# LiMeng95/MultiPoseNet.pytorch

Measured on AMD Instinct MI355X. Metric: images/sec (train fwd+bwd) ResNet101 480x480 bs=32/GPU, higher is better.
Workload: dtype bf16; 1 GPU; R101 full posenet (keypoint+detection) train step: fwd + MSE/focal losses + bwd + Adam, 480x480, 32 images/GPU, bf16 MFMA / fp32 accumulate / fp32 master weights; global_batch=32, parallelism=dp1, loss_log=asynchronous (set_lazy_log), launch=recorded launch list re-issued per step (replay.py), 87 replays, optimizer_update=Adam in one launch after backward

## Files before the change

### include/mpn.h

```cpp
#ifndef MPN_H_
#define MPN_H_
#include <stdint.h>

#ifdef __cplusplus
extern "C" {
#endif

#define MPN_F32 0
#define MPN_BF16 1
#define MPN_F16 2

#define MPN_E_BADARG (-2)
#define MPN_E_UNSUPPORTED (-3)

typedef struct MpnConvParams {
    const void* x;
    const void* w;
    void* y;
    const float* bias;
    const float* scale;
    const void* res;
    const uint8_t* res_mask;
    float* stats;
    int64_t x_sB, x_sH, x_sW;
// ... 51 lines not shown
    const void* dy;
    float* dw;
    float* ws;
    int64_t x_sB, x_sH, x_sW;
    int64_t dy_sP;
    int32_t B, H, W, Cin;
    int32_t Ho, Wo, Cout;
    int32_t R, S, stride, pad;
    int32_t dtype;
    int32_t chunks;
    float* db;
    float* db_ws;
    int32_t nseg;
    int32_t seg_H[5], seg_W[5];
    int32_t seg_chunk0[6];
    int32_t seg_chunk_pixels;
    const void* seg_x[5];
    const void* seg_dy[5];
    int32_t kseg_n, kseg_c;
    int32_t kseg_shift[4];
    const void* kseg_x[4];
} MpnWgradParams;
int mpn_debug_wgrad_prof(void* buf);
int mpn_debug_igemm_prof(void* buf);

int mpn_conv_wgrad_chunks(const MpnWgradParams* p);
int mpn_conv_wgrad_seg_plan(MpnWgradParams* p);
int mpn_conv_wgrad(const MpnWgradParams* p, void* stream);
int mpn_conv_wgrad_partials(const MpnWgradParams* p, void* stream);
int mpn_conv_wgrad_reduce(const MpnWgradParams* p, void* stream);
int mpn_conv_wgrad_kernel_id(const MpnWgradParams* p);
int mpn_conv_wgrad_kernel_name(const MpnWgradParams* p, char* buf, int cap);

int mpn_reduce_partials(const float* ws, int chunks, int64_t n, float* dst, int accumulate, void* stream);

int mpn_cast_f32_to_bf16(const float* src, void* dst, int64_t n, void* stream);
int mpn_cast_f32(const float* src, void* dst, int64_t n, int dtype, void* stream);
int mpn_weight_transpose(const float* w, void* wt, int Cout, int RS, int Cin, int Cout_pad,
                         int dtype, void* stream);
int mpn_weight_transpose_batched(const float* arena, void* dst, const int64_t* table, int nlayers, int64_t nblocks,
                                 int dtype, void* stream);
int mpn_weight_pad_k(const float* w, void* dst, int Cout, int K, int Kpad, int dtype, void* stream);
int mpn_stem_pack_weight(const float* w, void* packed, int Cout, int dtype, void* stream);
int mpn_stem_unpack_wgrad(const float* dpacked, float* dw, int Cout, void* stream);
int mpn_stem_pack_image(const float* img, int64_t sB, int64_t sC, int64_t sH, int64_t sW, void* dst,
                        int B, int H, int W, int dtype, void* stream);

int mpn_bn_finalize_train(const float* stats, int tiles, int C, int64_t count, const float* gamma,
                          const float* beta, float* running_mean, float* running_var, float momentum,
                          float eps, float* mean, float* invstd, float* scale, float* shift, void* stream);
int mpn_bn_finalize_eval(int C, const float* gamma, const float* beta, const float* running_mean,
                         const float* running_var, float eps, float* mean, float* invstd,
                         float* scale, float* shift, void* stream);
int mpn_bn_act_forward(const void* y, const void* res, void* z, const float* scale, const float* shift,
                       int64_t P, int C, int Cs, int relu, int dtype, uint8_t* mask, void* stream);
int mpn_bn_bwd_reduce(const void* dz, const void* z, const void* y, const float* mean, const float* invstd,
                      const float* mask_scale, const float* mask_shift, float* partial, int chunks, int64_t P, int C, int Cs, int relu, int dtype, void* stream);
int mpn_bn_bwd_finalize(const float* partial, int chunks, int C, int64_t count, const float* gamma, const float* mean,
                        const float* invstd, int train, float* dgamma, float* dbeta, float* coef, void* stream);
int mpn_bn_bwd_apply(const void* dz, const void* z, const void* y, const float* k1, const float* k2, const float* k3,
                     const float* mask_scale, const float* mask_shift, void* dy, void* dres, int dres_accumulate, int64_t P, int C, int Cs, int relu, int dtype,
                     const uint8_t* mask, void* stream);
int mpn_bn_bwd_chunks(int64_t P, int Cs, int dtype);

int mpn_maxpool3x3s2_forward(const void* x, void* y, uint8_t* idx, int B, int H, int W, int Cs,
                             int Ho, int Wo, int dtype, void* stream);
// ... 162 lines not shown
```

### multiposenet/pytorch_amd/_lib.py

```python
import ctypes
import os
import subprocess

import torch

_HERE = os.path.dirname(os.path.abspath(__file__))
LIB_PATH = os.path.join(_HERE, "libmpn_hip.so")
CSRC = os.path.join(_HERE, "csrc")

F32, BF16, F16 = 0, 1, 2


class MpnError(RuntimeError):
    pass


class ConvParams(ctypes.Structure):
    _fields_ = [
        ("x", ctypes.c_void_p), ("w", ctypes.c_void_p), ("y", ctypes.c_void_p),
        ("bias", ctypes.c_void_p), ("scale", ctypes.c_void_p), ("res", ctypes.c_void_p), ("res_mask", ctypes.c_void_p),
        ("stats", ctypes.c_void_p),
        ("x_sB", ctypes.c_int64), ("x_sH", ctypes.c_int64), ("x_sW", ctypes.c_int64),
        ("y_sB", ctypes.c_int64), ("y_sP", ctypes.c_int64),
        ("res_sB", ctypes.c_int64), ("res_sP", ctypes.c_int64),
# ... 29 lines not shown
        ("seg_chunk_pixels", ctypes.c_int32), ("seg_x", ctypes.c_void_p * 5), ("seg_dy", ctypes.c_void_p * 5),
        ("kseg_n", ctypes.c_int32), ("kseg_c", ctypes.c_int32), ("kseg_shift", ctypes.c_int32 * 4), ("kseg_x", ctypes.c_void_p * 4),
    ]


_vp, _i, _i64, _f = ctypes.c_void_p, ctypes.c_int, ctypes.c_int64, ctypes.c_float
_PC = ctypes.POINTER(ConvParams)
_PW = ctypes.POINTER(WgradParams)

SIGNATURES = {
    "mpn_gt_heatmaps": (_i, [_vp, _vp, _i, _i, _vp, _i, _i, ctypes.c_double, ctypes.c_double, _vp]),
    "mpn_augment_image": (_i, [_vp, _i64, _vp, _i, _vp, _i, _i, ctypes.POINTER(ctypes.c_float), _vp]),
    "mpn_augment_mask": (_i, [_vp, _i64, _vp, _i, _vp, _i, _i, _i, _i, _vp]),
    "mpn_prn_train_maps": (_i, [_vp, _vp, _vp, _vp, _i, _i, _i, ctypes.c_double, _vp, _vp, _vp, _vp, _vp, _vp]),
    "mpn_heatmap_peaks_workspace_bytes": (_i64, [_i, _i, _i, _i, _i]),
    "mpn_heatmap_peaks": (_i, [_vp, _i64, _i64, _i64, _i64, _i, _i, _i, _i, _f, ctypes.c_double, _i, _vp, _vp, _i, _vp, _vp]),
    "mpn_resize": (_i, [_vp, _i64, _i64, _i64, _i, _i, _i, _vp, _i, _i, _i, ctypes.c_double, ctypes.c_double, _vp]),
    "mpn_prn_build_maps": (_i, [_vp, _vp, _vp, _vp, _i, _i, _i, ctypes.c_double, _vp, _vp, _vp, _vp, _vp]),
    "mpn_prn_scores": (_i, [_vp, _vp, _i, _i, _i, _i, _vp, _vp, _vp]),
    "mpn_prn_scores_compact": (_i, [_vp, _vp, _i, _i, _i, _i, _i, _vp, _vp, _vp, _vp, _vp, _vp]),
    "mpn_prn_match_host": (_i, [_i, _vp, _vp, _vp, _vp, _vp, _vp, _vp, _i, _vp, _i, _i, _vp, _vp]),
    "mpn_conv_stats_tiles": (_i, [_PC]),
    "mpn_conv_kernel_name": (_i, [_PC, ctypes.c_char_p, _i]),
    "mpn_conv_forward": (_i, [_PC, _vp]),
    "mpn_debug_wgrad_prof": (_i, [_vp]),
    "mpn_debug_igemm_prof": (_i, [_vp]),
    "mpn_conv_wgrad_chunks": (_i, [_PW]),
    "mpn_conv_wgrad_seg_plan": (_i, [_PW]),
    "mpn_conv_wgrad": (_i, [_PW, _vp]),
    "mpn_conv_wgrad_partials": (_i, [_PW, _vp]),
    "mpn_conv_wgrad_reduce": (_i, [_PW, _vp]),
    "mpn_conv_wgrad_kernel_id": (_i, [_PW]),
    "mpn_conv_wgrad_kernel_name": (_i, [_PW, ctypes.c_char_p, _i]),
    "mpn_reduce_partials": (_i, [_vp, _i, _i64, _vp, _i, _vp]),
    "mpn_cast_f32_to_bf16": (_i, [_vp, _vp, _i64, _vp]),
    "mpn_cast_f32": (_i, [_vp, _vp, _i64, _i, _vp]),
    "mpn_weight_transpose": (_i, [_vp, _vp, _i, _i, _i, _i, _i, _vp]),
    "mpn_weight_transpose_batched": (_i, [_vp, _vp, _vp, _i, _i64, _i, _vp]),
    "mpn_weight_pad_k": (_i, [_vp, _vp, _i, _i, _i, _i, _vp]),
    "mpn_stem_pack_weight": (_i, [_vp, _vp, _i, _i, _vp]),
    "mpn_stem_unpack_wgrad": (_i, [_vp, _vp, _i, _vp]),
    "mpn_stem_pack_image": (_i, [_vp, _i64, _i64, _i64, _i64, _vp, _i, _i, _i, _i, _vp]),
    "mpn_bn_finalize_train": (_i, [_vp, _i, _i, _i64, _vp, _vp, _vp, _vp, _f, _f, _vp, _vp, _vp, _vp, _vp]),
    "mpn_bn_finalize_eval": (_i, [_i, _vp, _vp, _vp, _vp, _f, _vp, _vp, _vp, _vp, _vp]),
    "mpn_bn_act_forward": (_i, [_vp, _vp, _vp, _vp, _vp, _i64, _i, _i, _i, _i, _vp, _vp]),
    "mpn_bn_bwd_reduce": (_i, [_vp, _vp, _vp, _vp, _vp, _vp, _vp, _vp, _i, _i64, _i, _i, _i, _i, _vp]),
    "mpn_bn_bwd_finalize": (_i, [_vp, _i, _i, _i64, _vp, _vp, _vp, _i, _vp, _vp, _vp, _vp]),
    "mpn_bn_bwd_apply": (_i, [_vp, _vp, _vp, _vp, _vp, _vp, _vp, _vp, _vp, _vp, _i, _i64, _i, _i, _i, _i, _vp, _vp]),
    "mpn_bn_bwd_chunks": (_i, [_i64, _i, _i]),
    "mpn_maxpool3x3s2_forward": (_i, [_vp, _vp, _vp, _i, _i, _i, _i, _i, _i, _i, _vp]),
    "mpn_maxpool3x3s2_backward": (_i, [_vp, _vp, _vp, _i, _i, _i, _i, _i, _i, _i, _vp]),
    "mpn_upsample_nearest_backward": (_i, [_vp, _vp, _i, _i, _i, _i, _i, _i, _i, _i, _vp]),
    "mpn_upsample_nearest_slice": (_i, [_vp, _vp, _i, _i, _i, _i, _i, _i, _i, _i, _i, _vp]),
    "mpn_upsample_nearest_slice_backward": (_i, [_vp, _vp, _i, _i, _i, _i, _i, _i, _i, _i, _i, _vp]),
    "mpn_export_f32": (_i, [_vp, _i, _vp, _i, _i, _i, _i, _i, _i, _i, _i64, _i64, _vp]),
    "mpn_import_grad": (_i, [_vp, _i64, _i64, _vp, _i, _i, _i, _i, _i, _i, _i, _i, _vp]),
    "mpn_nchw_to_nhwc_f32": (_i, [_vp, _i64, _i64, _i64, _i64, _vp, _i, _i, _i, _i, _vp]),
    "mpn_det_pack": (_i, [_vp, _i, _vp, _i, _i64, _i, _i, _i64, _vp]),
    "mpn_det_unpack": (_i, [_vp, _vp, _i, _i, _i64, _i, _i, _i64, _vp]),
    "mpn_relu_forward": (_i, [_vp, _vp, _i64, _i, _vp]),
    "mpn_relu_backward": (_i, [_vp, _vp, _vp, _i64, _i, _i, _vp]),
    "mpn_add_inplace": (_i, [_vp, _vp, _i64, _i, _vp]),
    "mpn_channel_sum": (_i, [_vp, _i, _i64, _i, _i, _vp, _i, _vp]),
    "mpn_colsum_rows": (_i, [_vp, _i, _i64, _i, _i, _vp, _vp]),
    "mpn_channel_sum_chunks": (_i, [_i64, _i, _i]),
    "mpn_mse_chunks": (_i, [_i64]),
# ... 20 lines not shown
    "mpn_box_decode_clip": (_i, [_vp, _vp, _vp, _i, _i, _f, _f, _vp]),
    "mpn_box_decode_clip_ms": (_i, [_vp, _vp, _vp, _i, _i, _f, _f, ctypes.POINTER(ctypes.c_float), _vp]),
    "mpn_clip_boxes": (_i, [_vp, _i64, _f, _f, _vp]),
    "mpn_score_filter": (_i, [_vp, _vp, _i, _f, _vp, _vp, _vp, _vp]),
    "mpn_score_filter_batched": (_i, [_vp, _vp, _i, _i, _f, _vp, _vp, _vp, _vp]),
    "mpn_gather_dets_batched": (_i, [_vp, _i64, _vp, _i64, _vp, _i, _i, _vp, _vp, _i64, _vp]),
    "mpn_gather_class": (_i, [_vp, _vp, _i, _vp, _i64, _vp, _i, _i, _vp, _i64, _vp]),
    "mpn_nms_batched_workspace_bytes": (_i64, [_i, _i64]),
    "mpn_nms_batched": (_i, [_vp, _i64, _vp, _i, _i64, _f, _i, _vp, _i64, _vp, _vp, _vp]),
    "mpn_nms_batched_topk": (_i, [_vp, _i64, _vp, _i, _i64, _i64, _f, _i, _vp, _i64, _vp, _vp, _vp]),
    "mpn_nms_workspace_bytes": (_i64, [_i64]),
    "mpn_nms": (_i, [_vp, _i64, _f, _i, _vp, _vp, _vp, _vp]),
    "mpn_adam_step": (_i, [_vp, _vp, _vp, _vp, _i64, _f, _f, _f, _f, _f, _f, _f, _f, _vp]),
    "mpn_adam_advance": (_i, [_vp, _vp]),
    "mpn_adam_step_dev": (_i, [_vp, _vp, _vp, _vp, _i64, _vp, _vp]),
    "mpn_grad_absmax_workspace_bytes": (_i64, [_i64]),
    "mpn_grad_absmax_partial": (_i, [_vp, _i64, _vp, _vp]),
    "mpn_grad_clip_finalize": (_i, [_vp, _i64, _vp, _vp, _vp, _vp]),
    "mpn_adam_step_clip_dev": (_i, [_vp, _vp, _vp, _vp, _i64, _vp, _vp, _vp]),
    "mpn_scale_by_dev": (_i, [_vp, _i64, _vp, _vp]),
    "mpn_fill_f32": (_i, [_vp, _f, _i64, _vp]),
    "mpn_copy_bytes": (_i, [_vp, _vp, _i64, _vp]),
    "mpn_step_log": (_i, [_vp, _vp, _vp, _vp]),
    "mpn_conv2cls_comb_elems": (_i64, [_i, _i]),
    "mpn_conv2cls_combine": (_i, [_vp, _vp, _i, _i, _vp]),
    "mpn_conv2cls_expand": (_i, [_vp, _vp, _vp, _i, _i, _i, _i, _i, _vp]),
    "mpn_conv2cls_classsum": (_i, [_vp, _vp, _i, _i, _i, _i, _vp]),
    "mpn_conv2cls_pool": (_i, [_vp, _vp, _vp, _i, _i, _i, _i, _i, _vp]),
    "mpn_conv2cls_tapsum": (_i, [_vp, _vp, _i, _i, _i, _i, _i, _vp]),
    "mpn_conv2cls_fold": (_i, [_vp, _vp, _i, _i, _vp]),
    "mpn_version": (ctypes.c_char_p, []),
}

_COUNT_FUNCS = {"mpn_conv_stats_tiles", "mpn_conv_kernel_name", "mpn_conv_wgrad_chunks", "mpn_conv_wgrad_seg_plan", "mpn_conv_wgrad_kernel_id", "mpn_conv_wgrad_kernel_name", "mpn_bn_bwd_chunks", "mpn_channel_sum_chunks",
                "mpn_mse_chunks", "mpn_mse_train_blocks", "mpn_focal_blocks", "mpn_focal_mc_blocks", "mpn_bce_chunks", "mpn_nms_workspace_bytes", "mpn_nms_batched_workspace_bytes", "mpn_heatmap_peaks_workspace_bytes", "mpn_conv2cls_comb_elems", "mpn_grad_absmax_workspace_bytes", "mpn_version"}

_lib = None


def build(force=False):
    if force and os.path.exists(LIB_PATH):
        os.remove(LIB_PATH)
    subprocess.check_call(["make", "-s", "-j8", "-C", CSRC])
    if not os.path.exists(LIB_PATH):
        raise MpnError("build did not produce %s" % LIB_PATH)
    return LIB_PATH


def use_experiments_build():
    global LIB_PATH
    assert _lib is None, "call use_experiments_build() before anything loads the library"
    subprocess.check_call(["make", "-s", "-j8", "-C", CSRC, "experiments"])
    LIB_PATH = os.path.join(_HERE, "libmpn_hip_experiments.so")
    return LIB_PATH


def lib():
    global _lib
    if _lib is None:
        if not os.path.exists(LIB_PATH):
            raise MpnError("libmpn_hip.so not found at %s — run `python -c 'import __graft_entry__ as g; g.build()'` "
                           "(or `make -C %s`).  There is no CPU fallback." % (LIB_PATH, CSRC))
        L = ctypes.CDLL(LIB_PATH)
        for name, (res, args) in SIGNATURES.items():
            fn = getattr(L, name)
            fn.restype = res
            fn.argtypes = args
# ... 42 lines not shown
```

### multiposenet/pytorch_amd/csrc/conv_wgrad.hip

```cpp
#include "conv_dma.h"
#include <stdio.h>
#include <stdlib.h>

namespace {

template <typename T> struct Ones16;
template <> struct Ones16<bf16_t> { static constexpr unsigned kPair = 0x3F803F80u; };
template <> struct Ones16<f16_t> { static constexpr unsigned kPair = 0x3C003C00u; };
template <> struct Ones16<float> { static constexpr unsigned kPair = 0u; };

struct PixState {
    int b, ho, wo;
    __device__ __forceinline__ void init(long pix, int Ho, int Wo) {
        const unsigned hw = (unsigned)Ho * (unsigned)Wo;
        const unsigned px = (unsigned)pix;
        const unsigned bb = px / hw;
        const unsigned rem = px - bb * hw;
        const unsigned hh = rem / (unsigned)Wo;
        b = (int)bb; ho = (int)hh; wo = (int)(rem - hh * (unsigned)Wo);
    }
    __device__ __forceinline__ void advance(int n, int Ho, int Wo) {
        wo += n;
        while (wo >= Wo) { wo -= Wo; if (++ho == Ho) { ho = 0; ++b; } }
    }
// ... 212 lines not shown
    const long NW = (long)p.Cout * taps * p.Cin;
    float* __restrict__ dst = (p.chunks > 1) ? (p.ws + (long)chunk * NW) : p.dw;
    const bool add = (p.chunks == 1);
#pragma unroll
    for (int i = 0; i < C::MM; ++i) {
        const int ml = wm * C::WTM + i * 16 + (lane >> 4) * 4;
        const int cin = m0 + ml;
        if (cin >= p.Cin) continue;
#pragma unroll
        for (int j = 0; j < C::MN; ++j) {
            const int nl = wn * C::WTN + j * 16 + (lane & 15);
            const int cout = n0 + nl;
            if (cout >= p.Cout) continue;
            float* q = dst + ((long)cout * taps + tap) * p.Cin + cin;
            float4 v = make_float4(acc[i][j][0], acc[i][j][1], acc[i][j][2], acc[i][j][3]);
            if (add) {
                const float4 o = *reinterpret_cast<const float4*>(q);
                v.x += o.x; v.y += o.y; v.z += o.z; v.w += o.w;
            }
            *reinterpret_cast<float4*>(q) = v;
        }
    }
}

typedef __attribute__((ext_vector_type(4))) short s16x4_t;

template <int ROWB> __device__ __forceinline__ int dma_swz(int k) {
    return ROWB >= 256 ? 2 * ((k & 3) | (((k >> 3) & 1) << 2)) : 2 * (((k >> 1) & 1) | (((k >> 3) & 1) << 1));
}

template <typename T, int ROWB> __device__ __forceinline__ int dma_swz_t(int k) {
    if (sizeof(T) == 4) return (k & 3) << 2;
    return dma_swz<ROWB>(k);
}

template <typename T, int TM, int TN, bool SEG, bool PROF = false, bool LIN = false>
__device__ __forceinline__ void conv_wgrad_dma_body(const MpnWgradParams& pk, long chunk_pixels, unsigned long long* prof = nullptr) {
    const bool ablate_stores = (chunk_pixels >> 62) & 1;
    chunk_pixels &= ~(1L << 62);
    constexpr int ES = (int)sizeof(T), EV = 16 / ES;
    constexpr int KP = 64 / ES, NST = 3;
    constexpr int ROWA = TM * ES, ROWB = TN * ES;
    constexpr int A_BYTES = KP * ROWA, B_BYTES = KP * ROWB;
    constexpr int STAGE_BYTES = A_BYTES + B_BYTES;
    constexpr int QA = A_BYTES / 4096, QB = B_BYTES / 4096;
    constexpr int RPA = 1024 / ROWA, RPB = 1024 / ROWB;
    constexpr int MM = TM / 32, MN = TN / 32;
    static_assert((TM == 128 || TM == 64) && (TN == 128 || TN == 64), "tile widths");
    static_assert(ES == 2 || !SEG, "f32: single tensor");
    __shared__ __attribute__((aligned(16))) unsigned char lds[NST * STAGE_BYTES];
    const int tid = threadIdx.x, lane = tid & 63, wave = tid >> 6;
    const int wm = wave >> 1, wn = wave & 1;
    const int tilesM = (pk.Cin + TM - 1) / TM, tilesN = (pk.Cout + TN - 1) / TN;
    const int taps = pk.R * pk.S;
    int bid = xcd_remap(blockIdx.x, gridDim.x);
    const int tn = bid % tilesN; bid /= tilesN;
    const int tm = bid % tilesM; bid /= tilesM;
    const int tap = bid % taps; bid /= taps;
    const int chunk = bid;
    MpnWgradParams p = pk;
    int chunk_local = chunk;
    if (SEG) {
        int l = 0;
#pragma unroll
        for (int k = 1; k < 5; ++k) l += (k < pk.nseg && chunk >= pk.seg_chunk0[k]) ? 1 : 0;
        l = rfl(l);
// ... 80 lines not shown
            const int hi = a_px[q].ho * p.stride - p.pad + r, wi = a_px[q].wo * p.stride - p.pad + s;
            const bool ok = a_on[q] && (unsigned)hi < (unsigned)p.H && (unsigned)wi < (unsigned)p.W;
            const unsigned off = ((unsigned)a_px[q].b * (unsigned)p.x_sB + (unsigned)(hi >> vsh) * (unsigned)p.x_sH +
                                  (unsigned)(wi >> vsh) * (unsigned)p.x_sW + (unsigned)(a_chan[q] - vc0)) * (unsigned)ES;
            lds_dma16(ok ? off : DMA_OOB, rsrc_x, 0u, __builtin_amdgcn_readfirstlane(st + (wave_u * QA + q) * 1024u));
            a_px[q].advance_digits(adv_b, adv_h, adv_w, p.Ho, p.Wo);
        }
#pragma unroll
        for (int q = 0; q < QB; ++q)
            lds_dma16(b_voff[q], rsrc_dy, b_soff, __builtin_amdgcn_readfirstlane(st + A_BYTES + (wave_u * QB + q) * 1024u));
        b_soff += b_step;
        if constexpr (LIN) {
            if (halo) {
#pragma unroll
                for (int q = 0; q < QA; ++q) {
                    a_px[q].advance_digits(0, adv_h, adv_w, p.Ho, p.Wo);
                    const bool ok = (unsigned)(a_px[q].ho + dr) < (unsigned)p.H && (unsigned)(a_px[q].wo + dsx) < (unsigned)p.W;
                    a_sel[q] = ok ? (unsigned)a_chan[q] : DMA_OOB;
                }
            }
        }
    };

    const int g8 = (lane >> 4) * 8, li = lane & 15;
    const int piece_chunk = (li & 3) >> 1, piece_half = (li & 1) * 8;
    int a_row[2], a_swz[2], b_row[2], b_swz[2];
#pragma unroll
    for (int h = 0; h < 2; ++h) {
        const int k = g8 + 4 * h + (li >> 2);
        a_row[h] = k * ROWA; a_swz[h] = dma_swz<ROWA>(k);
        b_row[h] = k * ROWB; b_swz[h] = dma_swz<ROWB>(k);
    }
    auto frag = [&](const unsigned char* tile, const int (&row)[2], const int (&swz)[2], int c0) -> u32x4_t {
        const int lc = (c0 >> 3) + piece_chunk;
        s16x4_t lo = __builtin_amdgcn_ds_read_tr16_b64_v4i16(
            (__attribute__((address_space(3))) s16x4_t*)(tile + row[0] + ((lc ^ swz[0]) * 16) + piece_half));
        s16x4_t hi = __builtin_amdgcn_ds_read_tr16_b64_v4i16(
            (__attribute__((address_space(3))) s16x4_t*)(tile + row[1] + ((lc ^ swz[1]) * 16) + piece_half));
        struct { s16x4_t a, b; } pr = {lo, hi};
        return __builtin_bit_cast(u32x4_t, pr);
    };
    const bool do_bias = p.db != nullptr && tm == 0 && tap == 0 && wm == 0;
    f32x4_t accb[MN];
#pragma unroll
    for (int j = 0; j < MN; ++j) accb[j] = (f32x4_t){0.f, 0.f, 0.f, 0.f};
    auto compute = [&](unsigned stage) {
        const unsigned char* la = lds + stage * STAGE_BYTES;
        const unsigned char* lb = la + A_BYTES;
        if constexpr (ES == 4) {
#pragma unroll
            for (int kq = 0; kq < 4; ++kq) {
                const int krow = kq * 4 + (lane >> 4);
                const int key = (lane >> 4) << 2;
                float fa[MM], fb[MN];
#pragma unroll
                for (int i = 0; i < MM; ++i) {
                    const int c = wm * (TM / 2) + i * 16 + (lane & 15);
                    fa[i] = *reinterpret_cast<const float*>(la + krow * ROWA + (((c >> 2) ^ key) * 16) + (c & 3) * 4);
                }
#pragma unroll
                for (int j = 0; j < MN; ++j) {
                    const int c = wn * (TN / 2) + j * 16 + (lane & 15);
                    fb[j] = *reinterpret_cast<const float*>(lb + krow * ROWB + (((c >> 2) ^ key) * 16) + (c & 3) * 4);
                }
#pragma unroll
                for (int i = 0; i < MM; ++i)
#pragma unroll
                    for (int j = 0; j < MN; ++j)
                        acc[i][j] = __builtin_amdgcn_mfma_f32_16x16x4f32(fa[i], fb[j], acc[i][j], 0, 0, 0);
                if (do_bias) {
#pragma unroll
                    for (int j = 0; j < MN; ++j) accb[j] = __builtin_amdgcn_mfma_f32_16x16x4f32(1.0f, fb[j], accb[j], 0, 0, 0);
                }
// ... 260 lines not shown
        if (tm == 128 && tn == 128) hipLaunchKernelGGL((KERNEL<128, 128>), g, blk, 0, st, p, chunk_pixels);              \
        else if (tm == 128) hipLaunchKernelGGL((KERNEL<128, 64>), g, blk, 0, st, p, chunk_pixels);                       \
        else if (tn == 128) hipLaunchKernelGGL((KERNEL<64, 128>), g, blk, 0, st, p, chunk_pixels);                       \
        else hipLaunchKernelGGL((KERNEL<64, 64>), g, blk, 0, st, p, chunk_pixels)
    if (sizeof(T) == 4 && r.dma) {
        if (r.lin) { MPN_WGRAD_DMA_LAUNCH(conv_wgrad_dma_lin_f32_kernel); }
        else { MPN_WGRAD_DMA_LAUNCH(conv_wgrad_dma_f32_kernel); }
        rc = mpn_launch_status();
    } else if (sizeof(T) == 2 && r.dma) {
#if MPN_EXP
        if (g_wgrad_prof && !r.seg && p.dtype == MPN_BF16 && tm == 128 && tn == 128) {
            if (r.lin) hipLaunchKernelGGL((conv_wgrad_dma_lin_prof_kernel<128, 128>), g, blk, 0, st, p, chunk_pixels, g_wgrad_prof);
            else hipLaunchKernelGGL((conv_wgrad_dma_prof_kernel<128, 128>), g, blk, 0, st, p, chunk_pixels, g_wgrad_prof);
        } else
#endif
        if (r.lin) {
            if (p.dtype == MPN_F16) { MPN_WGRAD_DMA_LAUNCH(conv_wgrad_dma_lin_f16_kernel); }
            else { MPN_WGRAD_DMA_LAUNCH(conv_wgrad_dma_lin_kernel); }
        } else if (r.seg) {
            if (p.dtype == MPN_F16) { MPN_WGRAD_DMA_LAUNCH(conv_wgrad_dma_seg_f16_kernel); }
            else { MPN_WGRAD_DMA_LAUNCH(conv_wgrad_dma_seg_kernel); }
        } else if (p.dtype == MPN_F16) { MPN_WGRAD_DMA_LAUNCH(conv_wgrad_dma_f16_kernel); }
        else { MPN_WGRAD_DMA_LAUNCH(conv_wgrad_dma_kernel); }
#undef MPN_WGRAD_DMA_LAUNCH
        rc = mpn_launch_status();
    } else if (tm == 128) rc = launch_wgrad_n<T, 128>(p, tn, grid, chunk_pixels, st);
    else if (tm == 64) rc = launch_wgrad_n<T, 64>(p, tn, grid, chunk_pixels, st);
    else rc = launch_wgrad_n<T, 32>(p, tn, grid, chunk_pixels, st);
    if (rc != 0) return rc;
    if (p.chunks > 1 && reduce) rc = launch_wgrad_reduce(p, st);
    return rc;
}

}

extern "C" int mpn_debug_wgrad_prof(void* buf) {
#if MPN_EXP
    g_wgrad_prof = (unsigned long long*)buf;
    return 0;
#else
    (void)buf;
    return MPN_E_UNSUPPORTED;
#endif
}

extern "C" int mpn_conv_wgrad_seg_plan(MpnWgradParams* p) {
    if (!p || p->nseg <= 0 || p->nseg > 5) return MPN_E_BADARG;
    const int want = mpn_conv_wgrad_chunks(p);
    if (want < 1) return want;
    const long P = wgrad_total_pixels(*p);
    static const bool fit = mpn_tune("MPN_WGRAD_SEG_FIT", 0) != 0;
    long cp = 0;
    int c = 0;
    for (long w = want; w >= 1; --w) {
        cp = (P + w - 1) / w;
        cp = ((cp + 31) / 32) * 32;
        c = 0;
        for (int l = 0; l < p->nseg; ++l) {
            p->seg_chunk0[l] = c;
            const long pl = (long)p->B * p->seg_H[l] * p->seg_W[l];
            c += (int)((pl + cp - 1) / cp);
        }
        if (!fit || c <= want || c <= p->nseg) break;
    }
    p->seg_chunk0[p->nseg] = c;
    p->seg_chunk_pixels = (int)cp;
// ... 60 lines not shown
}

extern "C" int mpn_conv_wgrad_reduce(const MpnWgradParams* pp, void* stream) {
    if (!pp) return MPN_E_BADARG;
    const MpnWgradParams& p = *pp;
    MPN_CHECK_ARG(p.dw && p.ws && p.chunks > 1 && p.Cout > 0 && p.Cin > 0 && p.R > 0 && p.S > 0 && (!p.db || p.db_ws));
    return launch_wgrad_reduce(p, (hipStream_t)stream);
}

extern "C" int mpn_conv_wgrad_kernel_id(const MpnWgradParams* p) {
    if (!p) return MPN_E_BADARG;
    const WgradRoute r = wgrad_route(*p);
    return (r.tm << 16) | (r.tn << 4) | (r.lin ? 2 : 0) | (r.dma ? 1 : 0);
}

extern "C" int mpn_conv_wgrad_kernel_name(const MpnWgradParams* p, char* buf, int cap) {
    if (!p || !buf || cap <= 0 || !mpn_dtype_ok(p->dtype)) return MPN_E_BADARG;
    const WgradRoute r = wgrad_route(*p);
    const int n = r.dma ? snprintf(buf, (size_t)cap, "conv_wgrad_dma%s%s_kernel<%d, %d>", r.lin ? "_lin" : (r.seg ? "_seg" : ""),
                                   p->dtype == MPN_F16 ? "_f16" : (p->dtype == MPN_F32 ? "_f32" : ""), r.tm, r.tn)
                        : snprintf(buf, (size_t)cap, "conv_wgrad_kernel<%s, %d, %d>", mpn_type_name(p->dtype), r.tm, r.tn);
    return n < cap ? n : MPN_E_BADARG;
}

extern "C" int mpn_reduce_partials(const float* ws, int chunks, int64_t n, float* dst, int accumulate, void* stream) {
    MPN_CHECK_ARG(ws && dst && chunks >= 1 && n > 0);
    if (n <= 8192 && chunks >= 32) {
        hipLaunchKernelGGL(reduce_partials_small_kernel, dim3((unsigned)((n + 15) / 16)), dim3(256), 0, (hipStream_t)stream,
                           ws, chunks, (long)n, dst, accumulate);
        return mpn_launch_status();
    }
    return launch_reduce_partials(ws, chunks, (long)n, dst, accumulate, (hipStream_t)stream);
}
```

### multiposenet/pytorch_amd/engine.py

```python
import ctypes
import os

import torch

from . import ops
from ._lib import MpnError, call, gpu_op
from .ops import Act, round_up


class Ctx(object):

    def __init__(self, train):
        self.train = train
        self.tape = []
        self.grads = {}
        self.keep = []
        self.out_grads = {}
        self.wt = {}
        self.wt_buf = None
        self.uses = {}
        self.bn_train_ran = False
        self.side_keep = []
        self.wt_ready = None
        self.bnb = {}
# ... 22 lines not shown
        return self.grads.pop(id(act), None)


def num_classes(cm):
    cout = cm.output.weight.shape[0]
    if cout % 9 != 0 or cout == 0 or getattr(cm, "num_anchors", 9) != 9:
        raise MpnError("classificationModel: the output convolution has %d channels; the detector needs 9 anchors x K classes" % cout)
    return cout // 9


def _geom(layer):
    w = layer.weight
    if w.dim() == 2:
        return w.shape[0], w.shape[1], 1, 1, 1, 0
    return w.shape[0], w.shape[1], w.shape[2], w.shape[3], layer.stride[0], layer.padding[0]


class Engine(object):
    def __init__(self, model):
        self.m = model
        self._drop_calls = 0
        self._side = None
        self._wt_plan_cache = None
        self.overlap_wgrad = os.environ.get("MPN_SIDE_STREAM", "1") != "0"
        self.pyramid_towers = os.environ.get("MPN_PYRAMID_TOWERS", "1") != "0"
        self.fuse_bn_stats = os.environ.get("MPN_BN_FUSED_STATS", "1") != "0"
        self.fold_bn = os.environ.get("MPN_FOLD_BN", "1") != "0"
        self.fuse_bn_finalize = os.environ.get("MPN_BN_FUSED_FINALIZE", "1") != "0"
        self.det_pyramid_side = int(os.environ.get("MPN_DET_PYRAMID_SIDE", "2"))
        self.bn_mask_bits = os.environ.get("MPN_BN_MASK_BITS", "1") != "0"
        self.defer_shortcut_grad = os.environ.get("MPN_DEFER_SHORTCUT_GRAD", "1") != "0"
        self.virtual_concat = os.environ.get("MPN_VIRTUAL_CONCAT", "1") != "0"
        self.conv2_classes = os.environ.get("MPN_CONV2_CLASSES", "1") != "0"

    def side_stream(self, device):
        if not self.overlap_wgrad or device.type != "cuda":
            return None
        if self._side is None:
            self._side = torch.cuda.Stream(device=device)
        return self._side

    def _on_side(self, ctx, device, keep, fn, torch_ops=False, done_event=False):
        side = self.side_stream(device)
        if side is None:
            fn()
            return None
        ctx.side_keep.append(keep)
        ev = torch.cuda.Event()
        gpu_op(ev.record, torch.cuda.current_stream(device))
        gpu_op(side.wait_event, ev)
        if torch_ops:
            with torch.cuda.stream(side):
                fn()
        else:
            ops.push_stream(side)
            try:
                fn()
            finally:
                ops.pop_stream()
        if not done_event:
            return None
        done = torch.cuda.Event()
        gpu_op(done.record, side)
        return done

    @property
# ... 552 lines not shown
        return src

    def stem(self, ctx, img):
        f = self.m.fpn
        B, _, H, W = img.shape
        Hp, Wp = H + 6, W + 8
        img = img.detach()
        if img.dtype != torch.float32:
            img = img.float()
        packed = torch.empty((B, Hp, Wp, 4), dtype=self.cdt, device=img.device)
        call("mpn_stem_pack_image", ops.ptr(img), img.stride(0), img.stride(1), img.stride(2), img.stride(3), ops.ptr(packed),
             B, H, W, ops.dtype_code(self.cdt), ops.stream_ptr())
        xa = Act(packed, 4)
        w = f.conv1.weight
        wp = torch.empty((64, 7, 32), dtype=self.cdt, device=img.device)
        call("mpn_stem_pack_weight", ops.ptr(self.m._arena.data_seg(w)), ops.ptr(wp), 64, ops.dtype_code(self.cdt), ops.stream_ptr())
        Ho, Wo = ops.conv_out_hw(H, W, 7, 7, 2, 3)
        geom = (Hp, Wp, Hp * Wp * 4, Wp * 4, 4)
        bn_train = f.bn1.training
        if self.fold_bn and not ctx.train and not bn_train:
            bst = ops.bn_finalize_eval(f.bn1.weight.data, f.bn1.bias.data, f.bn1.running_mean, f.bn1.running_var, f.bn1.eps)
            z, _ = ops.conv_forward(xa, wp, 64, 7, 1, 2, 0, cin=32, x_geom=geom, out_hw=(Ho, Wo), scale=bst.scale, bias=bst.shift, act=1)
            return self.maxpool(ctx, z)
        y, st = ops.conv_forward(xa, wp, 64, 7, 1, 2, 0, cin=32, x_geom=geom, out_hw=(Ho, Wo), want_stats=bn_train,
                                 bn_fin=self._bn_fin(f.bn1) if bn_train else None)
        if ctx.train and w.requires_grad:
            y.needs_grad = True
            self._note_use(ctx, w)

            def bwd():
                dy = ctx.pop_grad(y)
                if dy is None:
                    return self._param_grads(ctx, f.conv1, None)
                dwp = torch.empty((64, 7, 32), dtype=torch.float32, device=img.device)

                def wgrad(dw, db, i):
                    call("mpn_fill_f32", ops.ptr(dwp), 0.0, dwp.numel(), ops.stream_ptr())
                    ops.conv_wgrad(xa, dy, dwp, 64, 7, 1, 2, 0, cin=32, x_geom=geom)
                    call("mpn_stem_unpack_wgrad", ops.ptr(dwp), ops.ptr(dw), 64, ops.stream_ptr())
                self._param_grads(ctx, f.conv1, (dy,), (xa, dy, dwp), wgrad)
            ctx.tape.append(bwd)
        z = self.bn(ctx, y, st, f.bn1, True)
        return self.maxpool(ctx, z)

    def conv_bn(self, ctx, x, conv, bn, relu, res=None):
        if self.fold_bn and not ctx.train and not bn.training:
            st = ops.bn_finalize_eval(bn.weight.data, bn.bias.data, bn.running_mean, bn.running_var, bn.eps)
            O, I, R, S, stride, pad = _geom(conv)
            act = (3 if res is not None else 1) if relu else 0
            y, _ = ops.conv_forward(x, self.w_fwd(conv), O, R, S, stride, pad, scale=st.scale, bias=st.shift, act=act,
                                    res=res, res_mode=1 if res is not None else 0)
            return y
        y, s = self.conv(ctx, x, conv, stats=bn.training, bn=bn)
        return self.bn(ctx, y, s, bn, relu, res=res)

    def bottleneck(self, ctx, x, blk):
        z1 = self.conv_bn(ctx, x, blk.conv1, blk.bn1, True)
        z2 = self.conv_bn(ctx, z1, blk.conv2, blk.bn2, True)
        sc = self.conv_bn(ctx, x, blk.downsample[0], blk.downsample[1], False) if len(blk.downsample) > 0 else x
        return self.conv_bn(ctx, z2, blk.conv3, blk.bn3, True, res=sc)

    def backbone(self, ctx, img):
        f = self.m.fpn
        c = self.stem(ctx, img)
        feats = []
        for layer in (f.layer1, f.layer2, f.layer3, f.layer4):
# ... 170 lines not shown
```

### multiposenet/pytorch_amd/ops.py

```python
import ctypes
import os

import torch

from . import _lib
from ._lib import BF16, F16, F32, ConvParams, WgradParams, call


def round_up(v, m):
    return (v + m - 1) // m * m


def dtype_code(dt):
    if dt == torch.float32:
        return F32
    if dt == torch.bfloat16:
        return BF16
    if dt == torch.float16:
        return F16
    raise _lib.MpnError("unsupported dtype %s" % dt)


_STREAM_OVERRIDE = []

# ... 566 lines not shown
        for c in (0, 1):
            ho, wo = (H - a + 1) // 2, (W - c + 1) // 2
            t = (B * ho * wo + tile_pixels - 1) // tile_pixels
            plan.append((a, c, ho, wo, t, tile0))
            tile0 += t
    return plan


def conv_wgrad(x, dy, dw, Cout, R, S, stride, pad, cin=None, x_geom=None, db=None):
    dev = x.t.device
    dt = x.t.dtype
    p = WgradParams()
    if x_geom is None:
        H, W = x.H, x.W
        sB, sH, sW = x.H * x.W * x.Cs, x.W * x.Cs, x.Cs
        Cin = cin if cin is not None else x.C
    else:
        H, W, sB, sH, sW = x_geom
        Cin = cin
    p.x, p.dy, p.dw = x.t.data_ptr(), dy.t.data_ptr(), dw.data_ptr()
    p.x_sB, p.x_sH, p.x_sW = sB, sH, sW
    p.dy_sP = dy.Cs
    p.B, p.H, p.W, p.Cin = x.B, H, W, Cin
    p.Ho, p.Wo, p.Cout = dy.H, dy.W, Cout
    p.R, p.S, p.stride, p.pad = R, S, stride, pad
    p.dtype = dtype_code(dt)
    fused_db = db is not None and bool(call("mpn_conv_wgrad_kernel_id", ctypes.byref(p)) & 1)
    _launch_wgrad(p, dev, db if fused_db else None, lambda: 2.0 * x.B * dy.H * dy.W * Cout * R * S * Cin,
                  lambda chunks: "wgrad %dx%d %d->%d @%dx%d s%d chunks=%d|%d" % (R, S, Cin, Cout, dy.H, dy.W, stride, chunks,
                                                                               (x.B * H * W * Cin + x.B * dy.H * dy.W * dy.Cs) * (2 if is16(dt) else 4)))
    return fused_db


def bias_grad(dy, db, C):
    v = 4 if dy.t.dtype == torch.float32 else 8
    g = dy.Cs // v
    if dy.P <= 256 or dy.Cs % v != 0 or (g & (g - 1)) != 0:
        call("mpn_colsum_rows", ptr(dy.t), dtype_code(dy.t.dtype), dy.P, C, dy.Cs, ptr(db), stream_ptr())
        return
    chunks = call("mpn_channel_sum_chunks", dy.P, dy.Cs, dtype_code(dy.t.dtype))
    ws = workspace(chunks * C * 4, dy.t.device, slot=2)
    call("mpn_channel_sum", ptr(dy.t), dtype_code(dy.t.dtype), dy.P, C, dy.Cs, ptr(ws), chunks, stream_ptr())
    call("mpn_reduce_partials", ptr(ws), chunks, C, ptr(db), 1, stream_ptr())


def weight_transpose(w_master, wt, Cout, RS, Cin, Cout_pad):
    call("mpn_weight_transpose", ptr(w_master), ptr(wt), Cout, RS, Cin, Cout_pad, dtype_code(wt.dtype), stream_ptr())


def cast_lowp(src, dst):
    call("mpn_cast_f32", ptr(src), ptr(dst), src.numel(), dtype_code(dst.dtype), stream_ptr())


_fin_counters = {}
FIN_MAX_TILES = int(os.environ.get("MPN_BN_FIN_MAX_TILES", "64"))
FIN_COUNTERS = 64


def fin_in_launch(tiles, Cout=2):
    return tiles <= FIN_MAX_TILES and Cout % 2 == 0


def fin_counters(device):
    key = (device, stream_handle() if device.type == "cuda" else 0)
    t = _fin_counters.get(key)
    if t is None:
# ... 289 lines not shown
```

Before: 890.3 images/sec.

## Add dedicated tiled stem 7x7 weight-gradient kernel writing unpacked dw directly

```diff
diff --git a/include/mpn.h b/include/mpn.h
--- a/include/mpn.h
+++ b/include/mpn.h
@@ -107,6 +107,11 @@
 int mpn_conv_wgrad_kernel_id(const MpnWgradParams* p);
 int mpn_conv_wgrad_kernel_name(const MpnWgradParams* p, char* buf, int cap);
 
+int mpn_stem_wgrad(const void* packed, const void* dy, float* dw, float* ws, int B, int H, int W, int chunks, int dtype,
+                   int stage, void* stream);
+int mpn_stem_wgrad_chunks(int B, int H, int W, int most);
+int mpn_stem_wgrad_kernel_name(int dtype, char* buf, int cap);
+
 int mpn_reduce_partials(const float* ws, int chunks, int64_t n, float* dst, int accumulate, void* stream);
 
 int mpn_cast_f32_to_bf16(const float* src, void* dst, int64_t n, void* stream);
diff --git a/multiposenet/pytorch_amd/_lib.py b/multiposenet/pytorch_amd/_lib.py
--- a/multiposenet/pytorch_amd/_lib.py
+++ b/multiposenet/pytorch_amd/_lib.py
@@ -85,6 +85,9 @@
     "mpn_conv_wgrad_reduce": (_i, [_PW, _vp]),
     "mpn_conv_wgrad_kernel_id": (_i, [_PW]),
     "mpn_conv_wgrad_kernel_name": (_i, [_PW, ctypes.c_char_p, _i]),
+    "mpn_stem_wgrad": (_i, [_vp, _vp, _vp, _vp, _i, _i, _i, _i, _i, _i, _vp]),
+    "mpn_stem_wgrad_chunks": (_i, [_i, _i, _i, _i]),
+    "mpn_stem_wgrad_kernel_name": (_i, [_i, ctypes.c_char_p, _i]),
     "mpn_reduce_partials": (_i, [_vp, _i, _i64, _vp, _i, _vp]),
     "mpn_cast_f32_to_bf16": (_i, [_vp, _vp, _i64, _vp]),
     "mpn_cast_f32": (_i, [_vp, _vp, _i64, _i, _vp]),
@@ -171,7 +174,7 @@
     "mpn_version": (ctypes.c_char_p, []),
 }
 
-_COUNT_FUNCS = {"mpn_conv_stats_tiles", "mpn_conv_kernel_name", "mpn_conv_wgrad_chunks", "mpn_conv_wgrad_seg_plan", "mpn_conv_wgrad_kernel_id", "mpn_conv_wgrad_kernel_name", "mpn_bn_bwd_chunks", "mpn_channel_sum_chunks",
+_COUNT_FUNCS = {"mpn_conv_stats_tiles", "mpn_conv_kernel_name", "mpn_conv_wgrad_chunks", "mpn_conv_wgrad_seg_plan", "mpn_conv_wgrad_kernel_id", "mpn_conv_wgrad_kernel_name", "mpn_stem_wgrad_chunks", "mpn_stem_wgrad_kernel_name", "mpn_bn_bwd_chunks", "mpn_channel_sum_chunks",
                 "mpn_mse_chunks", "mpn_mse_train_blocks", "mpn_focal_blocks", "mpn_focal_mc_blocks", "mpn_bce_chunks", "mpn_nms_workspace_bytes", "mpn_nms_batched_workspace_bytes", "mpn_heatmap_peaks_workspace_bytes", "mpn_conv2cls_comb_elems", "mpn_grad_absmax_workspace_bytes", "mpn_version"}
 
 _lib = None
diff --git a/multiposenet/pytorch_amd/csrc/conv_wgrad.hip b/multiposenet/pytorch_amd/csrc/conv_wgrad.hip
--- a/multiposenet/pytorch_amd/csrc/conv_wgrad.hip
+++ b/multiposenet/pytorch_amd/csrc/conv_wgrad.hip
@@ -268,6 +268,15 @@
 template <typename T, int ROWB> __device__ __forceinline__ int dma_swz_t(int k) {
     if (sizeof(T) == 4) return (k & 3) << 2;
     return dma_swz<ROWB>(k);
+}
+
+__device__ __forceinline__ u32x4_t tr_frag(const unsigned char* tile, const int (&row)[2], const int (&swz)[2], int lc, int piece_half) {
+    s16x4_t lo = __builtin_amdgcn_ds_read_tr16_b64_v4i16(
+        (__attribute__((address_space(3))) s16x4_t*)(tile + row[0] + ((lc ^ swz[0]) * 16) + piece_half));
+    s16x4_t hi = __builtin_amdgcn_ds_read_tr16_b64_v4i16(
+        (__attribute__((address_space(3))) s16x4_t*)(tile + row[1] + ((lc ^ swz[1]) * 16) + piece_half));
+    struct { s16x4_t a, b; } pr = {lo, hi};
+    return __builtin_bit_cast(u32x4_t, pr);
 }
 
 template <typename T, int TM, int TN, bool SEG, bool PROF = false, bool LIN = false>
@@ -414,13 +423,7 @@
         b_row[h] = k * ROWB; b_swz[h] = dma_swz<ROWB>(k);
     }
     auto frag = [&](const unsigned char* tile, const int (&row)[2], const int (&swz)[2], int c0) -> u32x4_t {
-        const int lc = (c0 >> 3) + piece_chunk;
-        s16x4_t lo = __builtin_amdgcn_ds_read_tr16_b64_v4i16(
-            (__attribute__((address_space(3))) s16x4_t*)(tile + row[0] + ((lc ^ swz[0]) * 16) + piece_half));
-        s16x4_t hi = __builtin_amdgcn_ds_read_tr16_b64_v4i16(
-            (__attribute__((address_space(3))) s16x4_t*)(tile + row[1] + ((lc ^ swz[1]) * 16) + piece_half));
-        struct { s16x4_t a, b; } pr = {lo, hi};
-        return __builtin_bit_cast(u32x4_t, pr);
+        return tr_frag(tile, row, swz, (c0 >> 3) + piece_chunk, piece_half);
     };
     const bool do_bias = p.db != nullptr && tm == 0 && tap == 0 && wm == 0;
     f32x4_t accb[MN];
@@ -747,6 +750,143 @@
     return rc;
 }
 
+
+constexpr int kStemN = 64 * 7 * 7 * 3;
+
+struct StemWgradArgs {
+    const void* x; const void* dy;
+    float* dw; float* ws;
+    int B, Hp, Wp, Ho, Wo, chunks;
+    long chunk_pixels;
+};
+
+template <typename T>
+__device__ __forceinline__ void stem_wgrad_body(const StemWgradArgs& p) {
+    constexpr int KP = 32, NST = 3, TM = 256, TN = 64;
+    constexpr int ROWA = TM * 2, ROWB = TN * 2;
+    constexpr int A_BYTES = KP * ROWA, B_BYTES = KP * ROWB;
+    constexpr int STAGE_BYTES = A_BYTES + B_BYTES;
+    constexpr int QA = A_BYTES / 4096, QB = B_BYTES / 4096;
+    constexpr int RPA = 1024 / ROWA, RPB = 1024 / ROWB;
+    constexpr int MM = 4, MN = 4;
+    static_assert(QB == 1 && sizeof(T) == 2, "16-bit operands");
+    __shared__ __attribute__((aligned(16))) unsigned char lds[NST * STAGE_BYTES];
+    const int tid = threadIdx.x, lane = tid & 63;
+    const unsigned wave_u = (unsigned)__builtin_amdgcn_readfirstlane(tid >> 6);
+    const int chunk = blockIdx.x;
+    const long P = (long)p.B * p.Ho * p.Wo;
+    const long k_begin = (long)chunk * p.chunk_pixels;
+    long k_end = k_begin + p.chunk_pixels; if (k_end > P) k_end = P;
+    const long span = k_end - k_begin;
+    const int nsteps = span > 0 ? (int)((span + KP - 1) / KP) : 0;
+
+    const i32x4_t rsrc_x = make_rsrc(p.x, (unsigned)((long)p.B * p.Hp * p.Wp * 8));
+    const i32x4_t rsrc_dy = make_rsrc(p.dy, (unsigned)((span > 0 ? k_end : 0) * (long)ROWB));
+    const unsigned lds_base = (unsigned)(size_t)(__attribute__((address_space(3))) unsigned char*)lds;
+
+    unsigned a_lane[QA], a_pix[QA]; bool a_live[QA]; PixState a_px[QA];
+#pragma unroll
+    for (int q = 0; q < QA; ++q) {
+        const int row = ((int)wave_u * QA + q) * RPA + lane / (ROWA / 16);
+        const int j = (lane % (ROWA / 16)) ^ dma_swz<ROWA>(row);
+        const int tap = j >> 2;
+        a_live[q] = tap < 7;
+        a_lane[q] = (unsigned)(tap * p.Wp * 8 + (j & 3) * 16);
+        long pix = k_begin + row; if (pix > P) pix = P;
+        a_pix[q] = (unsigned)pix;
+        a_px[q].init(pix, p.Ho, p.Wo);
+    }
+    unsigned b_voff;
+    {
+        const int row = (int)wave_u * RPB + lane / (ROWB / 16);
+        const int chan = ((lane % (ROWB / 16)) ^ dma_swz<ROWB>(row)) * 8;
+        b_voff = (unsigned)(((k_begin + row) * (long)TN + chan) * 2);
+    }
+    const unsigned b_step = KP * ROWB;
+    unsigned b_soff = 0;
+    const unsigned kend_u = (unsigned)k_end;
+    const int adv_t = KP / p.Wo, adv_w = KP - adv_t * p.Wo, adv_b = adv_t / p.Ho, adv_h = adv_t - adv_b * p.Ho;
+
+    f32x4_t acc[MM][MN];
+#pragma unroll
+    for (int i = 0; i < MM; ++i)
+#pragma unroll
+        for (int j = 0; j < MN; ++j) acc[i][j] = (f32x4_t){0.f, 0.f, 0.f, 0.f};
+
+    auto issue = [&](unsigned stage) {
+        const unsigned st = lds_base + stage * STAGE_BYTES;
+#pragma unroll
+        for (int q = 0; q < QA; ++q) {
+            const bool ok = a_live[q] && a_pix[q] < kend_u;
+            const unsigned off = (((unsigned)a_px[q].b * (unsigned)p.Hp + 2u * (unsigned)a_px[q].ho) * (unsigned)p.Wp + 2u * (unsigned)a_px[q].wo) * 8u + a_lane[q];
+            lds_dma16(ok ? off : DMA_OOB, rsrc_x, 0u, __builtin_amdgcn_readfirstlane(st + (wave_u * QA + q) * 1024u));
+            a_px[q].advance_digits(adv_b, adv_h, adv_w, p.Ho, p.Wo);
+            a_pix[q] = a_pix[q] < kend_u ? a_pix[q] + KP : a_pix[q];
+        }
+        lds_dma16(b_voff, rsrc_dy, b_soff, __builtin_amdgcn_readfirstlane(st + A_BYTES + wave_u * 1024u));
+        b_soff += b_step;
+    };
+
+    const int g8 = (lane >> 4) * 8, li = lane & 15;
+    const int piece_chunk = (li & 3) >> 1, piece_half = (li & 1) * 8;
+    int a_row[2], a_swz[2], b_row[2], b_swz[2];
+#pragma unroll
+    for (int h = 0; h < 2; ++h) {
+        const int k = g8 + 4 * h + (li >> 2);
+        a_row[h] = k * ROWA; a_swz[h] = dma_swz<ROWA>(k);
+        b_row[h] = k * ROWB; b_swz[h] = dma_swz<ROWB>(k);
+    }
+    auto compute = [&](unsigned stage) {
+        const unsigned char* la = lds + stage * STAGE_BYTES;
+        const unsigned char* lb = la + A_BYTES;
+        u32x4_t fa[MM], fb[MN];
+#pragma unroll
+        for (int i = 0; i < MM; ++i) fa[i] = tr_frag(la, a_row, a_swz, (int)wave_u * 8 + i * 2 + piece_chunk, piece_half);
+#pragma unroll
+        for (int j = 0; j < MN; ++j) fb[j] = tr_frag(lb, b_row, b_swz, j * 2 + piece_chunk, piece_half);
+#pragma unroll
+        for (int i = 0; i < MM; ++i)
+#pragma unroll
+            for (int j = 0; j < MN; ++j)
+                Mma<T>::run(acc[i][j], fa[i], fb[j]);
+    };
+
+    issue(0u);
+    issue(1u);
+    unsigned cur = 0u, nxt = 2u;
+    for (int it = 0; it < nsteps; ++it) {
+        wait_vmcnt<QA + QB>();
+        __builtin_amdgcn_s_barrier();
+        issue(nxt);
+        compute(cur);
+        cur = (cur == NST - 1) ? 0u : cur + 1u;
+        nxt = (nxt == NST - 1) ? 0u : nxt + 1u;
+    }
+    wait_vmcnt<0>();
+
+    float* __restrict__ dst = (p.chunks > 1) ? (p.ws + (long)chunk * kStemN) : p.dw;
+    const bool add = (p.chunks == 1);
+#pragma unroll
+    for (int i = 0; i < MM; ++i) {
+        const int m = (int)wave_u * 64 + i * 16 + (lane >> 4) * 4;
+        const int tap = m >> 5, s = (m & 31) >> 2;
+        if (tap >= 7 || s >= 7) continue;
+#pragma unroll
+        for (int j = 0; j < MN; ++j) {
+            const int cout = j * 16 + (lane & 15);
+            float* q = dst + ((cout * 7 + tap) * 7 + s) * 3;
+#pragma unroll
+            for (int c = 0; c < 3; ++c) q[c] = (add ? q[c] : 0.f) + acc[i][j][c];
+        }
+    }
+}
+
+__global__ void __launch_bounds__(256, 2) stem_wgrad_kernel(const StemWgradArgs p) { stem_wgrad_body<bf16_t>(p); }
+__global__ void __launch_bounds__(256, 2) stem_wgrad_f16_kernel(const StemWgradArgs p) { stem_wgrad_body<f16_t>(p); }
+
+inline long stem_out_pixels(int B, int H, int W) { return (long)B * ((H - 1) / 2 + 1) * ((W - 1) / 2 + 1); }
+constexpr long kStemMaxChunks = 1024;
+
 }
 
 extern "C" int mpn_debug_wgrad_prof(void* buf) {
@@ -873,3 +1013,45 @@
     }
     return launch_reduce_partials(ws, chunks, (long)n, dst, accumulate, (hipStream_t)stream);
 }
+
+extern "C" int mpn_stem_wgrad_chunks(int B, int H, int W, int most) {
+    MPN_CHECK_ARG(B > 0 && H > 0 && W > 0);
+    const long P = stem_out_pixels(B, H, W);
+    const long ksteps = (P + 31) / 32;
+    if (most) return (int)(ksteps < kStemMaxChunks ? ksteps : kStemMaxChunks);
+    long want = (P + 511) / 512;
+    if (want > kWgradTarget) want = kWgradTarget;
+    const long cp = (((P + want - 1) / want + 31) / 32) * 32;
+    return (int)((P + cp - 1) / cp);
+}
+
+extern "C" int mpn_stem_wgrad(const void* packed, const void* dy, float* dw, float* ws, int B, int H, int W, int chunks, int dtype,
+                              int stage, void* stream) {
+    MPN_CHECK_ARG(packed && dy && dw && B > 0 && H > 0 && W > 0 && (dtype == MPN_BF16 || dtype == MPN_F16));
+    MPN_CHECK_ARG(chunks >= 1 && chunks <= mpn_stem_wgrad_chunks(B, H, W, 1) && (chunks == 1 || ws) && stage >= 0 && stage <= 2 && (stage == 0 || chunks > 1));
+    StemWgradArgs a;
+    a.x = packed; a.dy = dy; a.dw = dw; a.ws = ws;
+    a.B = B; a.Hp = H + 6; a.Wp = W + 8; a.Ho = (H - 1) / 2 + 1; a.Wo = (W - 1) / 2 + 1; a.chunks = chunks;
+    const long P = stem_out_pixels(B, H, W);
+    if ((long)B * a.Hp * a.Wp * 8 >= 0x7fffffffL || (P + 32 * 3) * 128 >= 0x7fffffffL) return MPN_E_UNSUPPORTED;
+    a.chunk_pixels = (((P + chunks - 1) / chunks + 31) / 32) * 32;
+    hipStream_t st = (hipStream_t)stream;
+    if (stage != 2) {
+        if (dtype == MPN_F16) hipLaunchKernelGGL(stem_wgrad_f16_kernel, dim3((unsigned)chunks), dim3(256), 0, st, a);
+        else hipLaunchKernelGGL(stem_wgrad_kernel, dim3((unsigned)chunks), dim3(256), 0, st, a);
+        const int rc = mpn_launch_status();
+        if (rc != 0) return rc;
+    }
+    if (chunks > 1 && stage != 1) {
+        hipLaunchKernelGGL(reduce_partials_small_kernel, dim3((unsigned)((kStemN + 15) / 16)), dim3(256), 0, st,
+                           (const float*)ws, chunks, (long)kStemN, dw, 1);
+        return mpn_launch_status();
+    }
+    return 0;
+}
+
+extern "C" int mpn_stem_wgrad_kernel_name(int dtype, char* buf, int cap) {
+    if (!buf || cap <= 0 || !(dtype == MPN_BF16 || dtype == MPN_F16)) return MPN_E_BADARG;
+    const int n = snprintf(buf, (size_t)cap, "stem_wgrad%s_kernel", dtype == MPN_F16 ? "_f16" : "");
+    return n < cap ? n : MPN_E_BADARG;
+}
diff --git a/multiposenet/pytorch_amd/engine.py b/multiposenet/pytorch_amd/engine.py
--- a/multiposenet/pytorch_amd/engine.py
+++ b/multiposenet/pytorch_amd/engine.py
@@ -78,6 +78,7 @@
         self.defer_shortcut_grad = os.environ.get("MPN_DEFER_SHORTCUT_GRAD", "1") != "0"
         self.virtual_concat = os.environ.get("MPN_VIRTUAL_CONCAT", "1") != "0"
         self.conv2_classes = os.environ.get("MPN_CONV2_CLASSES", "1") != "0"
+        self.stem_wgrad_tile = os.environ.get("MPN_STEM_WGRAD", "1") != "0"
 
     def side_stream(self, device):
         if not self.overlap_wgrad or device.type != "cuda":
@@ -696,6 +697,8 @@
                 dy = ctx.pop_grad(y)
                 if dy is None:
                     return self._param_grads(ctx, f.conv1, None)
+                if self.stem_wgrad_tile and ops.is16(self.cdt):
+                    return self._param_grads(ctx, f.conv1, (dy,), (xa, dy), lambda dw, db, i: ops.stem_wgrad(packed, dy, dw, H, W))
                 dwp = torch.empty((64, 7, 32), dtype=torch.float32, device=img.device)
 
                 def wgrad(dw, db, i):
diff --git a/multiposenet/pytorch_amd/ops.py b/multiposenet/pytorch_amd/ops.py
--- a/multiposenet/pytorch_amd/ops.py
+++ b/multiposenet/pytorch_amd/ops.py
@@ -622,6 +622,34 @@
     return fused_db
 
 
+def stem_wgrad(packed, dy, dw, H, W, chunks=None):
+    dt = packed.dtype
+    B = packed.shape[0]
+    assert is16(dt) and dy.t.dtype == dt and tuple(packed.shape) == (B, H + 6, W + 8, 4) and packed.is_contiguous()
+    assert (dy.B, dy.H, dy.W, dy.Cs) == (B, (H - 1) // 2 + 1, (W - 1) // 2 + 1, 64) and dy.t.is_contiguous()
+    if chunks is None:
+        chunks = call("mpn_stem_wgrad_chunks", B, H, W, 0)
+    if chunks < 1:
+        raise _lib.MpnError("mpn_stem_wgrad_chunks failed with status %d" % chunks)
+    ws = workspace(chunks * 64 * 147 * 4, packed.device, slot=1).data_ptr() if chunks > 1 else None
+    args = (ptr(packed), ptr(dy.t), ptr(dw), ws, B, H, W, chunks, dtype_code(dt))
+    if not KERNEL_EVENTS.on:
+        call("mpn_stem_wgrad", *(args + (0, stream_ptr())))
+        return
+    buf = ctypes.create_string_buffer(64)
+    n = call("mpn_stem_wgrad_kernel_name", dtype_code(dt), buf, len(buf))
+    if n < 0:
+        raise _lib.MpnError("mpn_stem_wgrad_kernel_name failed with status %d" % n)
+    name = buf.value.decode()
+    if KERNEL_EVENTS.detail:
+        name = "wgrad stem 7x7x3 (7 taps x 32)->64 @%dx%d s2 chunks=%d|%d" % (dy.H, dy.W, chunks, (packed.numel() + dy.t.numel()) * 2)
+    e0 = KERNEL_EVENTS.begin()
+    call("mpn_stem_wgrad", *(args + (1 if chunks > 1 else 0, stream_ptr())))
+    KERNEL_EVENTS.end(name, 2.0 * dy.P * 64 * 7 * 32, e0)
+    if chunks > 1:
+        call("mpn_stem_wgrad", *(args + (2, stream_ptr())))
+
+
 def bias_grad(dy, db, C):
     v = 4 if dy.t.dtype == torch.float32 else 8
     g = dy.Cs // v
```

Measured after the change: 894.9 images/sec, median of 6. Within noise of the previous version (+0.5%).
